# GRatTWCU/Social-STGCNN

Hardware: AMD Instinct MI355X
Metric: scene-windows/sec fwd+bwd (obs=8,pred=12) (higher is better)
Workload: dtype f32; 1 GPU; synthetic V=32 scene-windows, obs 8 / pred 12, batch 2048 per GPU, f32 (BASELINE north-star: V<=32, batch=2048; SURVEY 8d generator); global_batch=2048, step=aggregation + forward + bivariate NLL + backward + SGD update, parallelism=dp1

## Files before the change

social_stgcnn_amd/csrc/common.hpp:

```cpp
#pragma once
#include <hip/hip_runtime.h>
#include <cstdarg>
#include <cstdio>
#include <cstdint>

#include "../../include/stgcnn_hip.h"

namespace stg {

char *last_error_buf();
int fail(int code, const char *fmt, ...);
int hip_fail(hipError_t e, const char *what);

#define STG_REQUIRE(cond, code, ...)            \
    do {                                        \
        if (!(cond)) return stg::fail((code), __VA_ARGS__); \
    } while (0)

#define STG_LAUNCH_CHECK(what)                           \
    do {                                                 \
        hipError_t e_ = hipGetLastError();               \
        if (e_ != hipSuccess) return stg::hip_fail(e_, what); \
    } while (0)

static inline hipStream_t as_stream(void *s) { return reinterpret_cast<hipStream_t>(s); }
static inline bool aligned(const void *p, uintptr_t bytes) { return ((uintptr_t)p & (bytes - 1)) == 0; }

struct Launch {
    const char *what;
    dim3 grid, block;
    size_t lds;
    hipStream_t st;
    size_t raise_above = 0;
};
int raise_lds_limit(const void *kernel, size_t lds, const char *what);
template <typename... Params, typename... Args>
inline int launch(const Launch &l, void (*kernel)(Params...), const Args &...args) {
    if (l.lds > l.raise_above) {
        const int rc = raise_lds_limit(reinterpret_cast<const void *>(kernel), l.lds, l.what);
        if (rc != STG_OK) return rc;
    }
    hipLaunchKernelGGL(kernel, l.grid, l.block, l.lds, l.st, args...);
    STG_LAUNCH_CHECK(l.what);
    return STG_OK;
}

#ifdef STG_DIAG
int diag_env(const char *name, int dflt);
#define STG_SKIP(args, bit) (((args).debug_skip & (bit)) != 0)
#else
static inline int diag_env(const char *, int dflt) { return dflt; }
#define STG_SKIP(args, bit) false
#endif

__device__ __forceinline__ void stagger_start(int wave, int waves, int units) {
    if (waves >= 2 && wave >= waves / 2) {
        if (units == -1) __builtin_amdgcn_s_setprio(1);
        else if (units == -2) __builtin_amdgcn_s_setprio(2);
        else if (units <= -3) __builtin_amdgcn_s_setprio(3);
        for (int i = 0; i < units; ++i) __builtin_amdgcn_s_sleep(127);
    }
}

struct EventList {
    void **ev;
    int n, next;
    hipStream_t st;
    void mark() {
        if (ev && next < n) (void)hipEventRecord(reinterpret_cast<hipEvent_t>(ev[next]), st);
        ++next;
    }
    void finish() {
        while (ev && next < n) mark();
    }
};

constexpr int kWave = 64;
constexpr int kLdsBytes = 160 * 1024;
constexpr int kNumCU = 256;

template <int CTRL, int ROW_MASK = 0xf>
__device__ __forceinline__ void dpp_add(float &v) {
    v += __int_as_float(__builtin_amdgcn_update_dpp(0, __float_as_int(v), CTRL, ROW_MASK, 0xf, false));
}
__device__ __forceinline__ float wave_sum(float v) {
    dpp_add<0xB1>(v);
    dpp_add<0x4E>(v);
    dpp_add<0x141>(v);
    dpp_add<0x140>(v);
    dpp_add<0x142, 0xa>(v);
    dpp_add<0x143, 0xc>(v);
    return __int_as_float(__builtin_amdgcn_readlane(__float_as_int(v), 63));
}
template <int CTRL, int ROW_MASK = 0xf, int K>
__device__ __forceinline__ void dpp_stage(float (&v)[K]) {
#pragma unroll
    for (int k = 0; k < K; ++k) dpp_add<CTRL, ROW_MASK>(v[k]);
}
template <int K>
__device__ __forceinline__ void wave_sum_to_last(float (&v)[K]) {
    dpp_stage<0xB1>(v);
    dpp_stage<0x4E>(v);
    dpp_stage<0x141>(v);
    dpp_stage<0x140>(v);
    dpp_stage<0x142, 0xa>(v);
    dpp_stage<0x143, 0xc>(v);
}
template <int K>
__device__ __forceinline__ void wave_sum_n(float (&v)[K]) {
    wave_sum_to_last<K>(v);
#pragma unroll
    for (int k = 0; k < K; ++k) v[k] = __int_as_float(__builtin_amdgcn_readlane(__float_as_int(v[k]), 63));
}
__device__ __forceinline__ double wave_sum(double v) {
#pragma unroll
    for (int o = 32; o > 0; o >>= 1) v += __shfl_xor(v, o, 64);
    return v;
}

}
```

social_stgcnn_amd/csrc/scene_team.hpp:

```cpp
#pragma once
#include "common.hpp"

namespace stg {

__device__ __forceinline__ void team_barrier() { asm volatile("s_waitcnt lgkmcnt(0)\n\ts_barrier" ::: "memory"); }

struct SoloScene {
    static constexpr bool kTeam = false;
    int vi;
    __device__ __forceinline__ int w0() const { return 0; }
    __device__ __forceinline__ int wc() const { return vi; }
    __device__ __forceinline__ int nch() const { return 1; }
    __device__ __forceinline__ int ci() const { return 0; }
    __device__ __forceinline__ bool lead() const { return true; }
    __device__ __forceinline__ void sync() const { __builtin_amdgcn_wave_barrier(); }
    template <int K>
    __device__ __forceinline__ void sum(float (&v)[K], int) const { wave_sum_n<K>(v); }
    template <int K>
    __device__ __forceinline__ void reduce(float (&v)[K]) const { wave_sum_to_last<K>(v); }
    __device__ __forceinline__ bool writer() const { return (threadIdx.x & 63) == 63; }
    __device__ __forceinline__ float *row(float *scene_row) const { return scene_row; }
};

constexpr int kXrF_s1 = 0, kXrF_s2 = 20, kXrF_sm2 = 40, kXrF_sv2 = 80, kXrFwd = 120;
constexpr int kXrB_s1 = 0, kXrB_s3 = 64, kXrRows = 128;
constexpr int kTeamRow = 160;
constexpr int kTeamRowLoss = kTeamRow - 1;

struct TeamScene {
    static constexpr bool kTeam = true;
    int vi;
    int w0_, wc_;
    int nch_, ci_;
    float *xr;
    float *rows;
    bool bar;
    __device__ __forceinline__ int w0() const { return w0_; }
    __device__ __forceinline__ int wc() const { return wc_; }
    __device__ __forceinline__ int nch() const { return nch_; }
    __device__ __forceinline__ int ci() const { return ci_; }
    __device__ __forceinline__ bool lead() const { return ci_ == 0; }
    __device__ __forceinline__ void sync() const {
        if (bar) team_barrier();
        else __builtin_amdgcn_wave_barrier();
    }
    template <int K>
    __device__ __forceinline__ void sum(float (&v)[K], int slot) const {
        if (nch_ == 1) {
            wave_sum_n<K>(v);
            return;
        }
        wave_sum_to_last<K>(v);
        float *x = xr + slot;
        if ((threadIdx.x & 63) == 63) {
#pragma unroll
            for (int k = 0; k < K; ++k) x[ci_ * K + k] = v[k];
            if (nch_ == 2) {
#pragma unroll
                for (int k = 0; k < K; ++k) x[(ci_ + 2) * K + k] = 0.f;
            }
        }
        if (bar) team_barrier();
        float p[4][K];
#pragma unroll
        for (int c = 0; c < 4; ++c)
#pragma unroll
            for (int k = 0; k < K; ++k) p[c][k] = x[c * K + k];
#pragma unroll
        for (int k = 0; k < K; ++k) v[k] = (p[0][k] + p[1][k]) + (p[2][k] + p[3][k]);
    }
    template <int K>
    __device__ __forceinline__ void reduce(float (&v)[K]) const { wave_sum_to_last<K>(v); }
    __device__ __forceinline__ bool writer() const { return (threadIdx.x & 63) == 63; }
    __device__ __forceinline__ float *row(float *) const { return rows + ci_ * kTeamRow; }
    __device__ __forceinline__ const float *row_of(int c) const { return rows + c * kTeamRow; }
};

constexpr int kXrBwdWg = 2 * kXrRows + 4 * kTeamRow;

}
```

social_stgcnn_amd/csrc/txp_x6.hip:

```cpp
#include "txp_scene_common.hpp"
#include "nll_elem.hpp"
#include "txp_conv_bf16.hpp"

namespace stg {

namespace {

constexpr int C = Cfg::C, P = Cfg::P, T = Cfg::T;

constexpr int64_t kCanonAggStride32[2] = {(int64_t)(Cfg::CIN0 + 1) * Cfg::T * kCanonV, kCanonWs32};
constexpr int64_t kCanonAggAx32[2] = {0, kCanonLayout.ws_hdr_floats + (int64_t)kCanonLayout.blk[0].ws_ax * kCanonV};
constexpr int64_t kCanonAggCs32[2] = {(int64_t)Cfg::CIN0 * Cfg::T * kCanonV,
                                      kCanonLayout.ws_hdr_floats + (int64_t)kCanonLayout.blk[0].ws_cs * kCanonV};

template <Shape S, typename Args>
__device__ __forceinline__ void fold_shape(Args &a) {
    if constexpr (S != Shape::Generic) {
        ModelLayout k = kCanonLayout;
        k.eps = a.lay.eps;
        k.momentum = a.lay.momentum;
        k.bn_mode = a.lay.bn_mode;
        k.flags = a.lay.flags;
        k.wg_waves = a.lay.wg_waves;
        a.lay = k;
    }
    if constexpr (S == Shape::Canon32) {
        a.V = a.Vl = kCanonV;
        a.num_peds = nullptr;
        a.tier.order = nullptr;
        a.tier.key_start = nullptr;
        a.ws_stride = kCanonWs32;
    }
}
__device__ __forceinline__ unsigned canon32_code(int t, int nq) {
    return (unsigned)(cv::tile_row(kCanonV, t) << 8 | (cv::tile_col0(kCanonV, t) + nq));
}
template <Shape S>
__device__ __forceinline__ int lay_txp_b(const ModelLayout &L, int l) {
    if constexpr (S == Shape::Generic) return L.txp_b[l];
    else return kCanonLayout.txp_b[l];
}
template <Shape S>
__device__ __forceinline__ int lay_ws_z(const ModelLayout &L, int l) {
    if constexpr (S == Shape::Generic) return L.ws_z[l];
    else return kCanonLayout.ws_z[l];
}

#ifdef STG_DIAG
#define STG_X6_STAMP(a, n, k)                                                                                          \
    do {                                                                                                              \
        if ((a).stamps && (threadIdx.x & 63) == 0) (a).stamps[(int64_t)(n) * 16 + (k)] = __builtin_amdgcn_s_memrealtime(); \
    } while (0)
#else
#define STG_X6_STAMP(a, n, k) do { } while (0)
#endif

constexpr int kF6Tiles = 10, kF6Slots = 7;

__host__ __device__ inline int fwd6_region_floats(int v) { return (cv::image_bytes(v, kF6Slots) / 4 + 3) & ~3; }

template <bool BF, typename CK, Shape SH = Shape::Generic>
__device__ __forceinline__ void txp_fwd_scene_x6(const TxpFwdArgs &a, const float *__restrict__ params,
                                                 const float *blk_params, const float *blk_buffers, int n, int vi,
                                                 float *region, ptab_t *ptab, const CK &ck) {
    const ModelLayout &L = a.lay;
    const int V = a.V, lane = threadIdx.x & 63, nq = lane & 15, kq = lane >> 4;
    float *yn = a.y + (int64_t)n * (C * P) * V;
    if (vi < V)
        for (int e = lane + 64 * ck.ci(); e < C * P * (V - vi); e += 64 * ck.nch()) {
            const int r = e / (V - vi), w = vi + (e - r * (V - vi));
            yn[(int64_t)r * V + w] = 0.f;
        }
    if (vi == 0) return;
    const int npos = C * ck.wc(), ntiles = (npos + 15) >> 4;
    const float *Pm = params;
    float *wsn = a.ws ? a.ws + n * a.ws_stride : nullptr;
    float *statn = a.stats ? a.stats + (int64_t)n * L.stat_floats : nullptr;
    unsigned char *img = reinterpret_cast<unsigned char *>(region);
    const cv::LaneGeom lg = cv::lane_geom(vi, kF6Slots);
    constexpr bool bf16 = BF;
    const int SWs = save_sw(vi, bf16), VWs = save_vw(vi, bf16);

    {
        float sv[C * T / 2];
        const float *agn = a.agg + n * a.agg_stride;
        stgcn_block_fwd_cols<true, SH != Shape::Canon32>(a, blk_params, blk_buffers, L.blk[0], n, vi, wsn, statn,
                                                         agn + a.agg_ax, agn + a.agg_cs, nullptr, 0, region,
                                                         cv::image_bytes(vi, kF6Slots) >> 4, ptab, sv, ck);
        float *d2 = wsn ? wsn + ws_plane_off(L, V, 0) : nullptr;
        const int pl = lane & 31, pw = ck.w0() + pl, q = lane >> 5;
        if (pl < ck.wc()) {
#pragma unroll
            for (int row = 0; row < C; ++row) {
                const f32x4 v4 = {sv[row], sv[C + row], sv[2 * C + row], sv[3 * C + row]};
                cv::put4(img, (unsigned)(cv::pos_off(vi, 1 + row, pw) + 8 * q), lg.PL, v4);
                if (d2) {
                    store_vec4(d2, (row * SWs + pw + 1) * 3 + q, v4, bf16);
                    if (q == 0) store_vec4(d2, (row * SWs + pw + 1) * 3 + 2, f32x4{0.f, 0.f, 0.f, 0.f}, bf16);
                }
            }
        }
        if (wsn && lane < 2 * C * 3 && ck.lead()) {
            const int b = lane / 3, q = lane - b * 3, pos = (b >> 1) * SWs + ((b & 1) ? vi + 1 : 0);
            for (int l = 0; l <= L.L; ++l)
                store_vec4(wsn + ws_plane_off(L, V, l), pos * 3 + q, f32x4{0.f, 0.f, 0.f, 0.f}, bf16);
        }
    }
    ck.sync();

    if (STG_SKIP(a, 16)) return;
    const unsigned lds_base = (unsigned)(uintptr_t)img;
    [[maybe_unused]] cv::LaneBases lb;
    if constexpr (SH == Shape::Canon32) {
        static_assert(!CK::kTeam && 16 * kF6Tiles == C * kCanonV, "Canon32: one wave, ten full tiles");
        lb = cv::lane_bases(lds_base, lg, vi);
    }
    f32x4 av[kF6Tiles];
#pragma unroll
    for (int t = 0; t < kF6Tiles; ++t) av[t] = f32x4{0.f, 0.f, 0.f, 0.f};
    for (int l = 0; l <= L.L; ++l) {
        const bool is_out = l == L.L;
        cv::u32x4 w[cv::kWpVecs];
        cv::load_wp(a.wpf + (int64_t)l * cv::kWpDwords, w);
        const float *bias = Pm + (is_out ? L.out_b : lay_txp_b<SH>(L, l));
        f32x4 binit;
#pragma unroll
        for (int r = 0; r < 4; ++r) binit[r] = kq < 3 ? bias[4 * kq + r] : 0.f;
        const float alpha = is_out ? 0.f : Pm[L.prelus + l];
        float *zs = (wsn && !is_out) ? wsn + L.ws_hdr_floats + (int64_t)lay_ws_z<SH>(L, l) * V : nullptr;
        float *ps = (wsn && !is_out) ? wsn + ws_plane_off(L, V, l + 1) : nullptr;
        asm volatile("" ::"v"(w[0]), "v"(w[cv::kWpVecs - 1]), "v"(binit), "v"(alpha) : "memory");
        vm_drain();
        __builtin_amdgcn_s_setprio(1);
        auto finish = [&](int t, int h, int wc, bool ok, const f32x4 &z) __attribute__((always_inline)) {
            if (ok && kq < 3) {
                if (is_out) {
#pragma unroll
                    for (int r = 0; r < 4; ++r) yn[(int64_t)((4 * kq + r) * C + h) * V + wc] = z[r];
                } else {
                    f32x4 v4;
#pragma unroll
                    for (int r = 0; r < 4; ++r) v4[r] = (z[r] > 0.f ? z[r] : alpha * z[r]) + av[t][r];
                    av[t] = v4;
                    if (zs) {
                        store_vec4(zs, (h * VWs + wc) * 3 + kq, z, bf16);
                        store_vec4(ps, (h * SWs + wc + 1) * 3 + kq, v4, bf16);
                    }
                }
            }
        };
        if constexpr (SH == Shape::Canon32) {
            cv::for_tiles<kF6Tiles>([&](auto tc) __attribute__((always_inline)) {
                constexpr int t = decltype(tc)::value;
                cv::BHalf b;
                f32x4 z = binit;
                cv::load_b_half_imm<0, kCanonV, t>(lb, b);
                cv::mma_half<0>(w, b, z);
                cv::load_b_half_imm<1, kCanonV, t>(lb, b);
                cv::mma_half<1>(w, b, z);
                finish(t, cv::tile_row(kCanonV, t), cv::tile_col0(kCanonV, t) + nq, true, z);
            });
        } else {
            unsigned code = cv::tile_code(0, ptab, npos);
#pragma unroll
            for (int t = 0; t < kF6Tiles; ++t) {
                if (t < ntiles) {
                    const cv::Tile tl = cv::tile_from<1>(t, code, npos, lg, vi);
                    if (t + 1 < kF6Tiles) code = cv::tile_code(t + 1, ptab, npos);
                    cv::BHalf b;
                    f32x4 z = binit;
                    cv::load_b_half<0>(lds_base, tl, b);
                    cv::mma_half<0>(w, b, z);
                    cv::load_b_half<1>(lds_base, tl, b);
                    cv::mma_half<1>(w, b, z);
                    finish(t, tl.h, tl.w, tl.ok, z);
                }
            }
        }
        __builtin_amdgcn_s_setprio(0);
        if (is_out) break;
        ck.sync();
        unsigned codes[kF6Tiles];
#pragma unroll
        for (int t = 0; t < kF6Tiles; ++t) codes[t] = SH == Shape::Canon32 ? canon32_code(t, nq) : cv::tile_code(t, ptab, npos);
#pragma unroll
        for (int t = 0; t < kF6Tiles; ++t) {
            const int p = 16 * t + nq;
            if (p < npos && kq < 3) {
                const unsigned hw = codes[t];
                cv::put4(img, (unsigned)(cv::pos_off(vi, 1 + (int)(hw >> 8), (int)(hw & 0xffu)) + 8 * kq), lg.PL, av[t]);
            }
        }
        ck.sync();
    }
}

template <int WPB, bool BF, Shape S>
__global__ __launch_bounds__(WPB * 64, WPB == 8 ? 1 : 2) __attribute__((amdgpu_waves_per_eu(2, 2))) void txp_fwd_x6_kernel(
    const TxpFwdArgs a0, const float *__restrict__ params, const float *__restrict__ buffers) {
    extern __shared__ __attribute__((aligned(16))) float sm[];
    TxpFwdArgs a = a0;
    fold_shape<S>(a);
    if constexpr (S == Shape::Canon32) {
        const int w = a.ws != nullptr;
        a.agg_stride = kCanonAggStride32[w];
        a.agg_ax = kCanonAggAx32[w];
        a.agg_cs = kCanonAggCs32[w];
    }
    const int Vl = a.Vl, wave = threadIdx.x >> 6;
    const int per_wave = fwd6_region_floats(Vl) + ptab_floats(Vl);
    float *region = sm + wave * per_wave;
    ptab_t *ptab = reinterpret_cast<ptab_t *>(region + fwd6_region_floats(Vl));
    float *blk_p = sm + WPB * per_wave, *blk_b = blk_p + ((a.lay.n_blk_params + 3) & ~3);
    stage_block_params(a.lay, params, buffers, blk_p, blk_b, WPB * 64);
    const int gw = __builtin_amdgcn_readfirstlane(blockIdx.x * WPB + wave), nw = gridDim.x * WPB;
    int begin, end;
    tier_range(a.tier, a.N, a.V, begin, end);
    const int M = end - begin;
    for (int r = 0; r * nw < M; ++r) {
        const int it = walk_item(r, gw, nw, M, a.tier.order != nullptr && a.tier.serpentine);
        if (it < 0) continue;
        const int n = __builtin_amdgcn_readfirstlane(a.tier.order ? scene_index(a.tier.order[begin + it], a.N) : it);
        int vi = a.num_peds ? a.num_peds[n] : a.V;
        vi = __builtin_amdgcn_readfirstlane(vi < 0 ? 0 : (vi > a.V ? a.V : vi));
        STG_X6_STAMP(a, n, 0);
        txp_fwd_scene_x6<BF, SoloScene, S>(a, params, blk_p, blk_b, n, vi, region, ptab, SoloScene{vi});
        __builtin_amdgcn_wave_barrier();
        STG_X6_STAMP(a, n, 8);
    }
}

constexpr int kX6Tiles = 10;
constexpr int kX6Slots = 7;
__host__ __device__ inline int bwd6_region_floats(int v) {
    const int img = cv::image_bytes(v, kX6Slots) / 4, tail = (2 * C * (T + 2) + C * T) * v;
    return ((img > tail ? img : tail) + 3) & ~3;
}

template <bool BF, typename CK, Shape SH = Shape::Generic>
__device__ __forceinline__ void txp_bwd_scene_x6(const TxpBwdArgs &a, const float *blk_params, int n, int vi, float *region,
                                                 ptab_t *ptab, const CK &ck) {
    const ModelLayout &L = a.lay;
    const int V = a.V, lane = threadIdx.x & 63, nq = lane & 15, kq = lane >> 4;
    float *slope_row = a.rows + (int64_t)n * (L.n_blk_params + L.n_txp) + L.n_blk_params;
    if (vi == 0) {
        for (int e = lane; e < L.n_blk_params + L.n_txp; e += 64) slope_row[e - L.n_blk_params] = 0.f;
        if (a.nll_target && lane == 0) a.nll_losses[n] = 0.f;
        return;
    }
    const int npos = C * ck.wc(), ntiles = (npos + 15) >> 4;
    const float *Pm = a.params;
    const float *wsn = a.ws + n * a.ws_stride;
    const float *dyn = a.dy + (int64_t)n * (C * P) * V;
    float *prow = ck.row(slope_row - L.n_blk_params);
    if constexpr (CK::kTeam) {
        for (int e = lane; e < kTeamRow; e += 64) prow[e] = 0.f;
    }
    unsigned char *img = reinterpret_cast<unsigned char *>(region);
    const cv::LaneGeom lg = cv::lane_geom(vi, kX6Slots);
    constexpr bool bf16 = BF;
    const int VWs = save_vw(vi, bf16);
    auto tile_slots = [&](int t, int &rec, int &quad) {
        if constexpr (SH == Shape::Canon32) {
            const int h = cv::tile_row(kCanonV, t), w = cv::tile_col0(kCanonV, t) + nq;
            quad = (h * VWs + w) * 3 + kq;
            rec = cv::pos_off(vi, 1 + h, w) + 8 * kq;
        } else {
            const int p = 16 * t + nq;
            const unsigned hw = ptab[p < npos ? p : 0];
            const int h = (int)(hw >> 8), w = (int)(hw & 0xffu);
            quad = (h * VWs + w) * 3 + kq;
            rec = (p < npos && kq < 3) ? cv::pos_off(vi, 1 + h, w) + 8 * kq : -1;
        }
    };
    auto has_quad = [&](int rec) { return SH == Shape::Canon32 ? kq < 3 : rec >= 0; };
    {
        uint4 *z4 = reinterpret_cast<uint4 *>(img);
        for (int e = lane + 64 * ck.ci(); e < cv::image_bytes(vi, kX6Slots) >> 4; e += 64 * ck.nch()) z4[e] = make_uint4(0u, 0u, 0u, 0u);
    }
    [[maybe_unused]] cv::LaneBases lb;
    if constexpr (SH == Shape::Canon32) {
        static_assert(!CK::kTeam && 16 * kX6Tiles == C * kCanonV, "Canon32: one wave, ten full tiles");
        lb = cv::lane_bases((unsigned)(uintptr_t)img, lg, vi);
    } else {
        build_ptab(ptab, ck.w0(), ck.wc());
    }
    ck.sync();
    f32x4 dcur[kX6Tiles];
#pragma unroll
    for (int t = 0; t < kX6Tiles; ++t) dcur[t] = f32x4{0.f, 0.f, 0.f, 0.f};

    for (int l = L.L; l >= 0; --l) {
        float *dzo = a.dzg + ((int64_t)n * (L.L + 1) + l) * dz_slot(V);
        if (STG_SKIP(a, 512) || (l == L.L && STG_SKIP(a, 2048)) || (l != L.L && STG_SKIP(a, 4096))) {
        } else if (l == L.L) {
            const int wcw = ck.wc();
            const int vp = wcw <= 1 ? 1 : (wcw <= 2 ? 2 : (wcw <= 4 ? 4 : (wcw <= 8 ? 8 : (wcw <= 16 ? 16 : 32))));
            const int sh = __builtin_ctz(vp), rpi = 64 >> sh;
            const int sub = lane >> sh, wl = lane & (vp - 1), w = ck.w0() + wl;
            const bool okw = wl < wcw;
            float *S = reinterpret_cast<float *>(img + lg.PL);
            auto put1 = [&](int rc, float g) { S[rc * vi + w] = g; };
            if (a.nll_target) {
                const float *tn = a.nll_target + (int64_t)n * P * V * 2;
                const float inv_cnt = 1.0f / (float)(P * vi);
                const float gs = inv_cnt * (a.nll_weights ? a.nll_weights[n] : 1.f);
                float lacc = 0.f;
#pragma unroll 1
                for (int p0 = 0; p0 < P; p0 += rpi) {
                    const int p = p0 + sub;
                    if (okw && p < P) {
                        const float *q = dyn + (int64_t)p * V + w;
                        const float2 tg = *reinterpret_cast<const float2 *>(tn + ((int64_t)p * V + w) * 2);
                        float g[5];
#ifdef STG_DIAG
                        if (STG_SKIP(a, 1 << 21))
                            lacc += nll_elem_t<true>(q[0], q[(int64_t)P * V], q[(int64_t)2 * P * V], q[(int64_t)3 * P * V],
                                                     q[(int64_t)4 * P * V], tg.x, tg.y, true, g);
                        else
#endif
                        lacc += nll_elem(q[0], q[(int64_t)P * V], q[(int64_t)2 * P * V], q[(int64_t)3 * P * V],
                                         q[(int64_t)4 * P * V], tg.x, tg.y, true, g);
#pragma unroll
                        for (int f = 0; f < C; ++f) put1(f * P + p, g[f] * gs);
                    }
                }
                float ls[1] = {lacc};
                ck.template reduce<1>(ls);
                if (ck.writer()) {
                    if constexpr (CK::kTeam) prow[kTeamRowLoss] = ls[0];
                    else a.nll_losses[n] = ls[0] * inv_cnt;
                }
            } else {
                constexpr int U = 4;
#pragma unroll 1
                for (int r0 = 0; r0 < C * P; r0 += rpi * U) {
                    float dv[U];
#pragma unroll
                    for (int u = 0; u < U; ++u) {
                        const int row = r0 + u * rpi + sub;
                        dv[u] = (okw && row < C * P) ? dyn[(int64_t)row * V + w] : 0.f;
                    }
#pragma unroll
                    for (int u = 0; u < U; ++u) {
                        const int row = r0 + u * rpi + sub;
                        if (okw && row < C * P) put1(row, dv[u]);
                    }
                }
            }
            __builtin_amdgcn_wave_barrier();
            vm_drain();
            f32x4 (&qd)[kX6Tiles] = dcur;
#pragma unroll
            for (int t = 0; t < kX6Tiles; ++t) {
                const int p = 16 * t + nq;
                const unsigned hw = SH == Shape::Canon32 ? canon32_code(t, nq) : ptab[p < npos ? p : 0];
                const float *sq = S + ((4 * (kq < 3 ? kq : 0)) * C + (int)(hw >> 8)) * vi + (int)(hw & 0xffu);
                qd[t] = f32x4{sq[0], sq[C * vi], sq[2 * C * vi], sq[3 * C * vi]};
            }
            ck.sync();
            {
                uint4 *z4 = reinterpret_cast<uint4 *>(img + lg.PL);
                for (int e = lane + 64 * ck.ci(); e < (2 * lg.PL + 128) >> 4; e += 64 * ck.nch()) z4[e] = make_uint4(0u, 0u, 0u, 0u);
            }
            ck.sync();
            int rec[kX6Tiles], qv[kX6Tiles];
#pragma unroll
            for (int t = 0; t < kX6Tiles; ++t) tile_slots(t, rec[t], qv[t]);
#pragma unroll
            for (int t = 0; t < kX6Tiles; ++t) {
                if (has_quad(rec[t])) {
                    cv::put4(img, (unsigned)rec[t], lg.PL, qd[t]);
                    store_vec4(dzo, qv[t], qd[t], bf16);
                }
            }
        } else {
            const float *zl = wsn + L.ws_hdr_floats + (int64_t)lay_ws_z<SH>(L, l) * V;
            const float alpha = Pm[L.prelus + l];
            float slope_acc = 0.f;
            f32x4 zv[kX6Tiles];
            int rec[kX6Tiles], qv[kX6Tiles];
#pragma unroll
            for (int t = 0; t < kX6Tiles; ++t) tile_slots(t, rec[t], qv[t]);
#pragma unroll
            for (int t = 0; t < kX6Tiles; ++t)
                zv[t] = has_quad(rec[t]) ? load_vec4_raw(zl, qv[t], bf16) : f32x4{1.f, 1.f, 1.f, 1.f};
            asm volatile("" ::"v"(zv[0]), "v"(zv[1]), "v"(zv[2]), "v"(zv[3]), "v"(zv[4]), "v"(zv[5]), "v"(zv[6]), "v"(zv[7]),
                         "v"(zv[8]), "v"(zv[9]), "v"(alpha)
                         : "memory");
            vm_drain();
#pragma unroll
            for (int t = 0; t < kX6Tiles; ++t) {
                if (has_quad(rec[t])) {
                    f32x4 dzv;
                    const f32x4 zq = finish_vec4(zv[t], bf16);
#pragma unroll
                    for (int r = 0; r < 4; ++r) {
                        const float z = zq[r], d = dcur[t][r];
                        float dz = d;
                        if (!(z > 0.f)) {
                            dz = alpha * d;
                            slope_acc = fmaf(d, z, slope_acc);
                        }
                        dzv[r] = dz;
                    }
                    cv::put4(img, (unsigned)rec[t], lg.PL, dzv);
                    store_vec4(dzo, qv[t], dzv, bf16);
                }
            }
            float ss[1] = {slope_acc};
            ck.template reduce<1>(ss);
            if (ck.writer()) prow[L.n_blk_params + l] = ss[0];
        }
        ck.sync();
        if (!STG_SKIP(a, 1024)) {
            cv::u32x4 w[cv::kWpVecs];
            cv::load_wp(a.wp + (int64_t)l * cv::kWpDwords, w);
            asm volatile("" ::"v"(w[0]), "v"(w[cv::kWpVecs - 1]) : "memory");
            vm_drain();
            const unsigned lds_base = (unsigned)(uintptr_t)img;
            const bool keep = l != L.L && l != 0;
            const f32x4 zero = {0.f, 0.f, 0.f, 0.f};
            if constexpr (SH == Shape::Canon32) {
                cv::for_tiles<kX6Tiles>([&](auto tc) __attribute__((always_inline)) {
                    constexpr int t = decltype(tc)::value;
                    cv::BHalf b;
                    f32x4 acc = keep ? dcur[t] : zero;
                    cv::load_b_half_imm<0, kCanonV, t>(lb, b);
                    cv::mma_half<0>(w, b, acc);
                    cv::load_b_half_imm<1, kCanonV, t>(lb, b);
                    cv::mma_half<1>(w, b, acc);
                    dcur[t] = acc;
                });
            } else {
                unsigned code = cv::tile_code(0, ptab, npos);
#pragma unroll
                for (int t = 0; t < kX6Tiles; ++t) {
                    if (t < ntiles) {
                        const cv::Tile tl = cv::tile_from<1>(t, code, npos, lg, vi);
                        if (t + 1 < kX6Tiles) code = cv::tile_code(t + 1, ptab, npos);
                        cv::BHalf b;
                        f32x4 acc = keep ? dcur[t] : zero;
                        cv::load_b_half<0>(lds_base, tl, b);
                        cv::mma_half<0>(w, b, acc);
                        cv::load_b_half<1>(lds_base, tl, b);
                        cv::mma_half<1>(w, b, acc);
                        dcur[t] = acc;
                    }
                }
            }
        }
        ck.sync();
    }
    float *D = region;
#pragma unroll
    for (int t = 0; t < kX6Tiles; ++t) {
        const int p = 16 * t + nq;
        if (p < npos && kq < T / 4) {
            const unsigned hw = SH == Shape::Canon32 ? canon32_code(t, nq) : ptab[p];
            const int h = (int)(hw >> 8), ww = (int)(hw & 0xffu);
#pragma unroll
            for (int r = 0; r < 4; ++r) D[((4 * kq + r) * C + h) * vi + ww] = dcur[t][r];
        }
    }
    __builtin_amdgcn_wave_barrier();
    if constexpr (!CK::kTeam) {
        for (int e = L.L + lane; e < L.n_txp; e += 64) slope_row[e] = 0.f;
    }
    if (!STG_SKIP(a, 4))
        stgcn_block_bwd_cols<true>(a, blk_params, L.blk[0], n, vi, D, slope_row - L.n_blk_params, a.ws + n * a.ws_stride, ck);
    if constexpr (CK::kTeam) {
        ck.sync();
        if (ck.lead()) {
            float *row = slope_row - L.n_blk_params;
            const int nrow = L.n_blk_params + L.n_txp;
            for (int e0 = 0; e0 < kTeamRow; e0 += 64) {
                const int e = e0 + lane < kTeamRow ? e0 + lane : kTeamRow - 2;
                float t = ck.row_of(0)[e];
                for (int c = 1; c < ck.nch(); ++c) t += ck.row_of(c)[e];
                if (e < nrow) row[e] = t;
                if (e == kTeamRowLoss && a.nll_target) a.nll_losses[n] = t * (1.0f / (float)(P * vi));
            }
        }
    }
}

template <int WPB, bool BF, Shape S>
__global__ __launch_bounds__(WPB * 64, WPB == 8 ? 1 : 2) __attribute__((amdgpu_waves_per_eu(2, 2))) void txp_bwd_x6_kernel(
    const TxpBwdArgs a0) {
    extern __shared__ __attribute__((aligned(16))) float sm[];
    TxpBwdArgs a = a0;
    fold_shape<S>(a);
    const int Vl = a.Vl, wave = threadIdx.x >> 6;
    const int per_wave = bwd6_region_floats(Vl) + bwd_ptab_floats(Vl);
    float *region = sm + wave * per_wave;
    ptab_t *ptab = reinterpret_cast<ptab_t *>(region + bwd6_region_floats(Vl));
    float *blk_p = sm + WPB * per_wave;
    stage_block_params(a.lay, a.params, nullptr, blk_p, nullptr, WPB * 64);
    const int gw = __builtin_amdgcn_readfirstlane(blockIdx.x * WPB + wave), nw = gridDim.x * WPB;
    int begin, end;
    tier_range(a.tier, a.N, a.V, begin, end);
    const int M = end - begin;
    for (int r = 0; r * nw < M; ++r) {
        const int it = walk_item(r, gw, nw, M, a.tier.order != nullptr && a.tier.serpentine);
        if (it < 0) continue;
        const int n = __builtin_amdgcn_readfirstlane(a.tier.order ? scene_index(a.tier.order[begin + it], a.N) : it);
        int vi = a.num_peds ? a.num_peds[n] : a.V;
        vi = __builtin_amdgcn_readfirstlane(vi < 0 ? 0 : (vi > a.V ? a.V : vi));
        STG_X6_STAMP(a, n, 0);
        txp_bwd_scene_x6<BF, SoloScene, S>(a, blk_p, n, vi, region, ptab, SoloScene{vi});
        __builtin_amdgcn_wave_barrier();
        STG_X6_STAMP(a, n, 8);
    }
}

__host__ __device__ inline int step6_per_wave_floats(int v) {
    const int f = fwd6_region_floats(v) + ptab_floats(v), b = bwd6_region_floats(v) + bwd_ptab_floats(v);
    return f > b ? f : b;
}

template <int WPB, bool BF>
__global__ __launch_bounds__(WPB * 64, 2) __attribute__((amdgpu_waves_per_eu(2, 2))) void txp_step_x6_kernel(
    const TxpFwdArgs f0, const TxpBwdArgs b0) {
    constexpr Shape S = Shape::Canon32;
    extern __shared__ __attribute__((aligned(16))) float sm[];
    TxpFwdArgs f = f0;
    fold_shape<S>(f);
    f.agg_stride = kCanonAggStride32[1];
    f.agg_ax = kCanonAggAx32[1];
    f.agg_cs = kCanonAggCs32[1];
    TxpBwdArgs b = b0;
    fold_shape<S>(b);
    const int wave = threadIdx.x >> 6;
    const int per_wave = step6_per_wave_floats(kCanonV);
    float *region = sm + wave * per_wave;
    ptab_t *ptab = reinterpret_cast<ptab_t *>(region + bwd6_region_floats(kCanonV));
    float *blk_p = sm + WPB * per_wave, *blk_b = blk_p + ((kCanonLayout.n_blk_params + 3) & ~3);
    stage_block_params(f.lay, f.params, f.buffers, blk_p, blk_b, WPB * 64);
    const int n = __builtin_amdgcn_readfirstlane(blockIdx.x * WPB + wave);
    if (n >= f.N) return;
    STG_X6_STAMP(f, n, 0);
    txp_fwd_scene_x6<BF, SoloScene, S>(f, f.params, blk_p, blk_b, n, kCanonV, region, ptab, SoloScene{kCanonV});
    __builtin_amdgcn_fence(__ATOMIC_RELEASE, "wavefront");
    __builtin_amdgcn_wave_barrier();
    __builtin_amdgcn_fence(__ATOMIC_ACQUIRE, "wavefront");
    STG_X6_STAMP(f, n, 8);
    STG_X6_STAMP(b, n, 0);
    txp_bwd_scene_x6<BF, SoloScene, S>(b, blk_p, n, kCanonV, region, ptab, SoloScene{kCanonV});
    __builtin_amdgcn_wave_barrier();
    STG_X6_STAMP(b, n, 8);
}

struct TeamCount {
    int n4, n2, n1;
    int u4, u2, units;
    bool sorted;
};
__device__ __forceinline__ TeamCount team_count(const SceneTier &t, const TeamGeom &g, const int32_t *num_peds, int N, int V) {
    TeamCount c;
    c.sorted = t.order && t.key_start;
    if (c.sorted) {
        const int a4 = g.v2 < V ? t.key_start[V - g.v2] : 0, a2 = g.v1 < V ? t.key_start[V - g.v1] : 0;
        c.n4 = a4;
        c.n2 = a2 - a4;
        c.u2 = (c.n2 + 1) >> 1;
    } else {
        const bool pairs = !num_peds && V > g.v1 && V <= g.v2;
        c.n4 = (V > g.v1 && !pairs) ? N : 0;
        c.n2 = pairs ? N : 0;
        c.u2 = (c.n2 + 1) >> 1;
    }
    c.n1 = N - c.n4 - c.n2;
    c.u4 = c.n4;
    c.units = c.u4 + c.u2 + ((c.n1 + 3) >> 2);
    return c;
}
struct TeamUnit {
    int n, vi;
    int nch, ci, slot;
    int w0, wc;
};
__device__ __forceinline__ TeamUnit team_unit(const SceneTier &t, const TeamCount &c, const int32_t *__restrict__ num_peds,
                                              int N, int V, int u) {
    const int wave = __builtin_amdgcn_readfirstlane(threadIdx.x >> 6);
    TeamUnit q;
    int idx;
    if (u < c.u4) {
        q.nch = 4; q.slot = 0; q.ci = wave; idx = u;
    } else if (u < c.u4 + c.u2) {
        const int i0 = c.n4 + 2 * (u - c.u4);
        if (i0 + 1 < c.n4 + c.n2) { q.nch = 2; q.slot = wave >> 1; q.ci = wave & 1; idx = i0 + q.slot; }
        else { q.nch = 4; q.slot = 0; q.ci = wave; idx = i0; }
    } else {
        q.nch = 1; q.slot = wave; q.ci = 0; idx = c.n4 + c.n2 + 4 * (u - c.u4 - c.u2) + wave;
    }
    q.n = idx < N ? (c.sorted ? scene_index(t.order[idx], N) : idx) : -1;
    q.n = __builtin_amdgcn_readfirstlane(q.n);
    int vi = q.n >= 0 ? (num_peds ? num_peds[q.n] : V) : 0;
    vi = __builtin_amdgcn_readfirstlane(vi < 0 ? 0 : (vi > V ? V : vi));
    q.vi = vi;
    const int wc = (vi + q.nch - 1) / q.nch;
    q.w0 = q.ci * wc;
    q.wc = vi - q.w0 < wc ? (vi - q.w0 > 0 ? vi - q.w0 : 0) : wc;
    return q;
}
__device__ __forceinline__ int team_workers(int units, int grid) {
    const int rounds = (units + grid - 1) / grid;
    return rounds > 0 ? (units + rounds - 1) / rounds : 1;
}
__host__ __device__ inline int team_ptab_floats() { return ptab_floats(32); }

template <bool BF>
__global__ __launch_bounds__(256, 2) __attribute__((amdgpu_waves_per_eu(2, 2))) void txp_fwd_team_kernel(
    const TxpFwdArgs a, const float *__restrict__ params, const float *__restrict__ buffers) {
    extern __shared__ __attribute__((aligned(16))) float sm[];
    const int wave = __builtin_amdgcn_readfirstlane(threadIdx.x >> 6);
    const int R = a.team.region_floats;
    ptab_t *ptab = reinterpret_cast<ptab_t *>(sm + R + wave * team_ptab_floats());
    float *xr = sm + R + 4 * team_ptab_floats();
    float *blk_p = xr + 2 * kXrFwd, *blk_b = blk_p + ((a.lay.n_blk_params + 3) & ~3);
    stage_block_params(a.lay, params, buffers, blk_p, blk_b, 256);
    const TeamCount tc = team_count(a.tier, a.team, a.num_peds, a.N, a.V);
    const int G = team_workers(tc.units, gridDim.x);
    int prev = 1;
    for (int r = 0; r * G < tc.units; ++r) {
        const int u = walk_item(r, blockIdx.x, G, tc.units, a.tier.serpentine != 0);
        if (u < 0 || (int)blockIdx.x >= G) continue;
        const TeamUnit q = team_unit(a.tier, tc, a.num_peds, a.N, a.V, u);
        if (q.nch > 1 || prev > 1) team_barrier();
        prev = q.nch;
        if (q.n >= 0) {
            const TeamScene ck{q.vi, q.w0, q.wc, q.nch, q.ci, xr + (q.slot & 1) * kXrFwd, nullptr, q.nch > 1 && !STG_SKIP(a, 1 << 20)};
            float *region = sm + q.slot * ((R >> 2) * q.nch);
            txp_fwd_scene_x6<BF>(a, params, blk_p, blk_b, q.n, q.vi, region, ptab, ck);
        }
        __builtin_amdgcn_wave_barrier();
    }
}

template <bool BF>
__global__ __launch_bounds__(256, 2) __attribute__((amdgpu_waves_per_eu(2, 2))) void txp_bwd_team_kernel(const TxpBwdArgs a) {
    extern __shared__ __attribute__((aligned(16))) float sm[];
    const int wave = __builtin_amdgcn_readfirstlane(threadIdx.x >> 6);
    const int R = a.team.region_floats;
    ptab_t *ptab = reinterpret_cast<ptab_t *>(sm + R + wave * team_ptab_floats());
    float *xr = sm + R + 4 * team_ptab_floats();
    float *blk_p = xr + kXrBwdWg;
    stage_block_params(a.lay, a.params, nullptr, blk_p, nullptr, 256);
    const TeamCount tc = team_count(a.tier, a.team, a.num_peds, a.N, a.V);
    const int G = team_workers(tc.units, gridDim.x);
    int prev = 1;
    for (int r = 0; r * G < tc.units; ++r) {
        const int u = walk_item(r, blockIdx.x, G, tc.units, a.tier.serpentine != 0);
        if (u < 0 || (int)blockIdx.x >= G) continue;
        const TeamUnit q = team_unit(a.tier, tc, a.num_peds, a.N, a.V, u);
        if (q.nch > 1 || prev > 1) team_barrier();
        prev = q.nch;
        if (q.n >= 0) {
            const TeamScene ck{q.vi, q.w0, q.wc, q.nch, q.ci, xr + (q.slot & 1) * kXrRows,
                               xr + 2 * kXrRows + q.slot * q.nch * kTeamRow, q.nch > 1 && !STG_SKIP(a, 1 << 20)};
            float *region = sm + q.slot * ((R >> 2) * q.nch);
            txp_bwd_scene_x6<BF>(a, blk_p, q.n, q.vi, region, ptab, ck);
        }
        __builtin_amdgcn_wave_barrier();
    }
}

}

bool txp_fwd_x6_fits(const ModelLayout &L, int V) {
    return L.n_txp > 0 && V <= kTeamMaxV && !(L.flags & STG_OPT_F32_MFMA) && L.n_blocks == 1 &&
           L.blk[0].cin == Cfg::CIN0 && !diag_env("STG_FWD_F32", 0);
}

constexpr int kTeamFineBatch = 1536, kTeamFinestBatch = 384;
static int team_waves(int v, int v1, int v2) { return v <= v1 ? 1 : (v <= v2 ? 2 : 4); }
static bool team_geom(int N, int V, bool uniform, TeamGeom *g) {
    g->on = 0;
    if (V > kTeamMaxV) return false;
    int v1 = 32, v2 = 64;
    if (N < kTeamFinestBatch) { v1 = 8; v2 = 16; }
    else if (N < kTeamFineBatch) { v1 = 16; v2 = 32; }
    if (uniform)
        while (v1 < 32 && (int64_t)N * team_waves(V, v1, v2) > 2048) { v1 *= 2; v2 *= 2; }
    if (const int e = diag_env("STG_TEAM_V1", 0)) v1 = e;
    if (const int e = diag_env("STG_TEAM_V2", 0)) v2 = e;
    if (v1 > 32) v1 = 32;
    if (v2 > 64) v2 = 64;
    if (v2 < v1) v2 = v1;
    auto region = [&](int v) { return fwd6_region_floats(v); };
    int r = 4 * region(v1 < V ? v1 : V);
    if (2 * region(v2 < V ? v2 : V) > r) r = 2 * region(v2 < V ? v2 : V);
    if (region(V) > r) r = region(V);
    g->on = 1; g->v1 = v1; g->v2 = v2; g->region_floats = (r + 15) & ~15;
    return true;
}
static bool team_wanted(int N, int V, bool uniform, TeamGeom *g) {
    if (!team_geom(N, V, uniform, g)) return false;
    return V > 16 * kF6Tiles / C || g->v1 < V || diag_env("STG_TEAM", 0) != 0;
}
static int team_grid(size_t lds_bytes, int N) {
    int per_cu = (int)(kLdsBytes / lds_bytes);
    if (per_cu > 2) per_cu = 2;
    if (per_cu < 1) per_cu = 1;
    const int g = kNumCU * per_cu;
    return g < N ? g : N;
}

template <typename Args>
static Shape canon_shape(const Args &a, bool *ok) {
    *ok = true;
    if (!is_canonical(a.lay)) return Shape::Generic;
    if (a.num_peds || a.V != kCanonV) return Shape::Canon;
    *ok = a.Vl == kCanonV && !a.tier.order && !a.tier.key_start && a.ws_stride == kCanonWs32;
    return Shape::Canon32;
}
static bool canon32_agg_matches(const TxpFwdArgs &a) {
    const int w = a.ws != nullptr;
    return a.agg_stride == kCanonAggStride32[w] && a.agg_ax == kCanonAggAx32[w] && a.agg_cs == kCanonAggCs32[w];
}

template <int W>
static auto fwd_x6_kernel(bool bf, Shape sh) {
    if (bf) return sh == Shape::Canon32 ? txp_fwd_x6_kernel<W, true, Shape::Canon32> : txp_fwd_x6_kernel<W, true, Shape::Generic>;
    if (sh == Shape::Canon32) return txp_fwd_x6_kernel<W, false, Shape::Canon32>;
    return sh == Shape::Canon ? txp_fwd_x6_kernel<W, false, Shape::Canon> : txp_fwd_x6_kernel<W, false, Shape::Generic>;
}
template <int W>
static auto bwd_x6_kernel(bool bf, Shape sh) {
    if (bf) {
        if (sh == Shape::Canon32) return txp_bwd_x6_kernel<W, true, Shape::Canon32>;
        return sh == Shape::Canon ? txp_bwd_x6_kernel<W, true, Shape::Canon> : txp_bwd_x6_kernel<W, true, Shape::Generic>;
    }
    if (sh == Shape::Canon32) return txp_bwd_x6_kernel<W, false, Shape::Canon32>;
    return sh == Shape::Canon ? txp_bwd_x6_kernel<W, false, Shape::Canon> : txp_bwd_x6_kernel<W, false, Shape::Generic>;
}

int launch_txp_fwd_x6(const TxpFwdArgs &a0, hipStream_t st) {
    TxpFwdArgs a = a0;
    STG_REQUIRE(a.wpf, STG_EINVAL, "txp_fwd_x6: the prepared operands are missing");
    const bool bf = (a.lay.flags & STG_OPT_BF16_STORE) != 0;
    if (team_wanted(a.N, a.V, a.num_peds == nullptr, &a.team)) {
        const size_t lds = ((size_t)a.team.region_floats + 4 * team_ptab_floats() + 2 * kXrFwd + wave_param_floats(a.lay)) * sizeof(float);
        STG_REQUIRE(lds <= (size_t)kLdsBytes, STG_ELDS, "txp_fwd_team: V=%d needs %zu bytes of LDS", a.V, lds);
        return launch(Launch{"txp_fwd_team", dim3(team_grid(lds, a.N)), dim3(256), lds, st},
                      bf ? txp_fwd_team_kernel<true> : txp_fwd_team_kernel<false>, a, a.params, a.buffers);
    }
    STG_REQUIRE(a.V <= 16 * kF6Tiles / C, STG_EUNSUPPORTED, "txp_fwd_x6: V=%d outside the exact-bf16 kernels", a.V);
    const size_t per_wave = (size_t)(fwd6_region_floats(a.Vl) + ptab_floats(a.Vl)) * sizeof(float);
    const int wpb = wave_wpb(per_wave) == 8 ? 8 : 4;
    const size_t lds = per_wave * wpb + wave_param_floats(a.lay) * sizeof(float);
    bool ok;
    const Shape sh = canon_shape(a, &ok);
    STG_REQUIRE(ok && (sh != Shape::Canon32 || canon32_agg_matches(a)), STG_EINVAL,
                "txp_fwd_x6: the canonical V=%d batch does not match its compiled layout", a.V);
    return launch(Launch{"txp_fwd_x6", dim3(wave_grid(lds, wpb, a.N)), dim3(wpb * 64), lds, st},
                  wpb == 8 ? fwd_x6_kernel<8>(bf, sh) : fwd_x6_kernel<4>(bf, sh), a, a.params, a.buffers);
}

bool txp_bwd_x6_fits(const ModelLayout &L, int V) {
    return L.n_txp > 0 && V <= kTeamMaxV && L.n_blocks == 1 && L.blk[0].cin == Cfg::CIN0 &&
           !(L.flags & (STG_OPT_SPLIT_BF16 | STG_OPT_F32_MFMA)) && !diag_env("STG_BWD_F32", 0);
}
int64_t txp_bwd_x6_wp_floats(const ModelLayout &L) { return (int64_t)(L.L + 1) * cv::kWpDwords; }
int launch_txp_bwd_x6(const TxpBwdArgs &a0, hipStream_t st) {
    TxpBwdArgs a = a0;
    STG_REQUIRE(a.wp, STG_EINVAL, "txp_bwd_x6: the prepared operands are missing");
    const bool bf = (a.lay.flags & STG_OPT_BF16_STORE) != 0;
    if (team_wanted(a.N, a.V, a.num_peds == nullptr, &a.team)) {
        const size_t lds = ((size_t)a.team.region_floats + 4 * team_ptab_floats() + kXrBwdWg + wave_param_floats(a.lay)) * sizeof(float);
        STG_REQUIRE(lds <= (size_t)kLdsBytes, STG_ELDS, "txp_bwd_team: V=%d needs %zu bytes of LDS", a.V, lds);
        return launch(Launch{"txp_bwd_team", dim3(team_grid(lds, a.N)), dim3(256), lds, st},
                      bf ? txp_bwd_team_kernel<true> : txp_bwd_team_kernel<false>, a);
    }
    STG_REQUIRE(a.V <= 16 * kX6Tiles / C, STG_EUNSUPPORTED, "txp_bwd_x6: V=%d outside the exact-bf16 kernels", a.V);
    const size_t per_wave = (size_t)(bwd6_region_floats(a.Vl) + bwd_ptab_floats(a.Vl)) * sizeof(float);
    const int wpb = wave_wpb(per_wave) == 8 ? 8 : 4;
    const size_t lds = per_wave * wpb + wave_param_floats(a.lay) * sizeof(float);
    bool ok;
    const Shape sh = canon_shape(a, &ok);
    STG_REQUIRE(ok, STG_EINVAL, "txp_bwd_x6: the canonical V=%d batch does not match its compiled layout", a.V);
    return launch(Launch{"txp_bwd_x6", dim3(wave_grid(lds, wpb, a.N)), dim3(wpb * 64), lds, st},
                  wpb == 8 ? bwd_x6_kernel<8>(bf, sh) : bwd_x6_kernel<4>(bf, sh), a);
}

static bool step_x6_plain(int debug_skip_f, int debug_skip_b, int stagger_f, int stagger_b) {
    const size_t pf = (size_t)(fwd6_region_floats(kCanonV) + ptab_floats(kCanonV)) * sizeof(float);
    const size_t pb = (size_t)(bwd6_region_floats(kCanonV) + bwd_ptab_floats(kCanonV)) * sizeof(float);
    return !debug_skip_f && !debug_skip_b && !stagger_f && !stagger_b && wave_wpb(pf) != 8 && wave_wpb(pb) != 8;
}
bool txp_step_x6_fits(const ModelLayout &L, const int32_t *num_peds, int N, int V) {
    TeamGeom g;
    const int skip = diag_env("STG_DEBUG_SKIP", 0);
    return is_canonical(L) && V == kCanonV && !num_peds && txp_fwd_x6_fits(L, V) && txp_bwd_x6_fits(L, V) &&
           !team_wanted(N, V, true, &g) &&
           step_x6_plain(skip, skip, diag_env("STG_STAGGER_F", 0), diag_env("STG_STAGGER_B", 0));
}
static bool txp_step_x6_applies(const TxpFwdArgs &f, const TxpBwdArgs &b) {
    if (!f.wpf || !b.wp || !f.ws || f.ws != b.ws || f.N != b.N || f.V != b.V || f.params != b.params) return false;
    if (f.lay.flags != b.lay.flags || !step_x6_plain(f.debug_skip, b.debug_skip, f.stagger, b.stagger)) return false;
    TeamGeom g;
    if (team_wanted(f.N, f.V, f.num_peds == nullptr, &g) || team_wanted(b.N, b.V, b.num_peds == nullptr, &g)) return false;
    bool okf, okb;
    if (canon_shape(f, &okf) != Shape::Canon32 || canon_shape(b, &okb) != Shape::Canon32) return false;
    return okf && okb && canon32_agg_matches(f);
}
int launch_txp_step_x6(const TxpFwdArgs &f, const TxpBwdArgs &b, hipStream_t st) {
    STG_REQUIRE(txp_step_x6_applies(f, b), STG_EINVAL, "txp_step_x6: the batch is outside the one-launch scene kernel");
    constexpr int wpb = 4;
    const size_t lds = ((size_t)step6_per_wave_floats(kCanonV) * wpb + wave_param_floats(f.lay)) * sizeof(float);
    const bool bf = (f.lay.flags & STG_OPT_BF16_STORE) != 0;
    STG_REQUIRE(2 * lds <= (size_t)kLdsBytes, STG_ELDS, "txp_step_x6: %zu bytes of LDS do not fit two workgroups per CU", lds);
    return launch(Launch{"txp_step_x6", dim3((f.N + wpb - 1) / wpb), dim3(wpb * 64), lds, st},
                  bf ? txp_step_x6_kernel<wpb, true> : txp_step_x6_kernel<wpb, false>, f, b);
}

}
```

Baseline: 10.86 million scene-windows/s.

## Hand off forward outputs through LDS in fused step kernel; inline-asm DPP wave sums

In the one-launch Canon32 step kernel, the forward pass now also writes its output tile into the LDS scratch image. The backward pass reads predictions from there for the NLL gradient instead of re-reading them from global memory, and only zeroes the part of the image it still needs. Separately, wave reductions for Canon32 solo scenes use hand-written batched v_add_f32_dpp inline assembly with a single s_nop per stage rather than per-value builtins. The assembly path relies on correct hazard padding, and the hand-off assumes P is even and that LDS regions do not overlap.

```diff
diff --git a/social_stgcnn_amd/csrc/common.hpp b/social_stgcnn_amd/csrc/common.hpp
--- a/social_stgcnn_amd/csrc/common.hpp
+++ b/social_stgcnn_amd/csrc/common.hpp
@@ -97,18 +97,83 @@
 #pragma unroll
     for (int k = 0; k < K; ++k) dpp_add<CTRL, ROW_MASK>(v[k]);
 }
-template <int K>
+#define STG_DPP_I(i, c) "v_add_f32_dpp %" #i ", %" #i ", %" #i " " c "\n\t"
+#define STG_DPP_I1(c) STG_DPP_I(0, c)
+#define STG_DPP_I5(c) STG_DPP_I1(c) STG_DPP_I(1, c) STG_DPP_I(2, c) STG_DPP_I(3, c) STG_DPP_I(4, c)
+#define STG_DPP_I10(c) STG_DPP_I5(c) STG_DPP_I(5, c) STG_DPP_I(6, c) STG_DPP_I(7, c) STG_DPP_I(8, c) STG_DPP_I(9, c)
+#define STG_DPP_I15(c) STG_DPP_I10(c) STG_DPP_I(10, c) STG_DPP_I(11, c) STG_DPP_I(12, c) STG_DPP_I(13, c) STG_DPP_I(14, c)
+#define STG_DPP_I16(c) STG_DPP_I15(c) STG_DPP_I(15, c)
+#define STG_DPP_I25(c)                                                                                               \
+    STG_DPP_I16(c) STG_DPP_I(16, c) STG_DPP_I(17, c) STG_DPP_I(18, c) STG_DPP_I(19, c) STG_DPP_I(20, c) STG_DPP_I(21, c) \
+        STG_DPP_I(22, c) STG_DPP_I(23, c) STG_DPP_I(24, c)
+#define STG_DPP_V(v, i) "+v"((v)[O + (i)])
+#define STG_DPP_V1(v) STG_DPP_V(v, 0)
+#define STG_DPP_V5(v) STG_DPP_V1(v), STG_DPP_V(v, 1), STG_DPP_V(v, 2), STG_DPP_V(v, 3), STG_DPP_V(v, 4)
+#define STG_DPP_V10(v) STG_DPP_V5(v), STG_DPP_V(v, 5), STG_DPP_V(v, 6), STG_DPP_V(v, 7), STG_DPP_V(v, 8), STG_DPP_V(v, 9)
+#define STG_DPP_V15(v) STG_DPP_V10(v), STG_DPP_V(v, 10), STG_DPP_V(v, 11), STG_DPP_V(v, 12), STG_DPP_V(v, 13), STG_DPP_V(v, 14)
+#define STG_DPP_V16(v) STG_DPP_V15(v), STG_DPP_V(v, 15)
+#define STG_DPP_V25(v)                                                                                               \
+    STG_DPP_V16(v), STG_DPP_V(v, 16), STG_DPP_V(v, 17), STG_DPP_V(v, 18), STG_DPP_V(v, 19), STG_DPP_V(v, 20), STG_DPP_V(v, 21), \
+        STG_DPP_V(v, 22), STG_DPP_V(v, 23), STG_DPP_V(v, 24)
+#define STG_DPP_STMT(v, c)                                                       \
+    do {                                                                         \
+        if constexpr (N == 25) asm("s_nop 1\n\t" STG_DPP_I25(c) : STG_DPP_V25(v)); \
+        else if constexpr (N == 16) asm("s_nop 1\n\t" STG_DPP_I16(c) : STG_DPP_V16(v)); \
+        else if constexpr (N == 15) asm("s_nop 1\n\t" STG_DPP_I15(c) : STG_DPP_V15(v)); \
+        else if constexpr (N == 10) asm("s_nop 1\n\t" STG_DPP_I10(c) : STG_DPP_V10(v)); \
+        else if constexpr (N == 5) asm("s_nop 1\n\t" STG_DPP_I5(c) : STG_DPP_V5(v)); \
+        else asm("s_nop 1\n\t" STG_DPP_I1(c) : STG_DPP_V1(v));                   \
+    } while (0)
+template <int S, int O = 0, int K>
+__device__ __forceinline__ void wave_sum_stage(float (&v)[K]) {
+    constexpr int R = K - O;
+    constexpr int N = R >= 25 ? 25 : (R >= 16 ? 16 : (R >= 15 ? 15 : (R >= 10 ? 10 : (R >= 5 ? 5 : 1))));
+    static_assert(S >= 0 && S < 6 && R >= 1, "six stages, at least one value");
+    if constexpr (S == 0) STG_DPP_STMT(v, "quad_perm:[1,0,3,2] row_mask:0xf bank_mask:0xf");
+    else if constexpr (S == 1) STG_DPP_STMT(v, "quad_perm:[2,3,0,1] row_mask:0xf bank_mask:0xf");
+    else if constexpr (S == 2) STG_DPP_STMT(v, "row_half_mirror row_mask:0xf bank_mask:0xf");
+    else if constexpr (S == 3) STG_DPP_STMT(v, "row_mirror row_mask:0xf bank_mask:0xf");
+    else if constexpr (S == 4) STG_DPP_STMT(v, "row_bcast:15 row_mask:0xa bank_mask:0xf");
+    else STG_DPP_STMT(v, "row_bcast:31 row_mask:0xc bank_mask:0xf");
+    if constexpr (R > N) wave_sum_stage<S, O + N>(v);
+}
+#undef STG_DPP_STMT
+#undef STG_DPP_V25
+#undef STG_DPP_V16
+#undef STG_DPP_V15
+#undef STG_DPP_V10
+#undef STG_DPP_V5
+#undef STG_DPP_V1
+#undef STG_DPP_V
+#undef STG_DPP_I25
+#undef STG_DPP_I16
+#undef STG_DPP_I15
+#undef STG_DPP_I10
+#undef STG_DPP_I5
+#undef STG_DPP_I1
+#undef STG_DPP_I
+
+template <int K, bool ASM = false>
 __device__ __forceinline__ void wave_sum_to_last(float (&v)[K]) {
-    dpp_stage<0xB1>(v);
-    dpp_stage<0x4E>(v);
-    dpp_stage<0x141>(v);
-    dpp_stage<0x140>(v);
-    dpp_stage<0x142, 0xa>(v);
-    dpp_stage<0x143, 0xc>(v);
+    if constexpr (ASM) {
+        wave_sum_stage<0>(v);
+        wave_sum_stage<1>(v);
+        wave_sum_stage<2>(v);
+        wave_sum_stage<3>(v);
+        wave_sum_stage<4>(v);
+        wave_sum_stage<5>(v);
+    } else {
+        dpp_stage<0xB1>(v);
+        dpp_stage<0x4E>(v);
+        dpp_stage<0x141>(v);
+        dpp_stage<0x140>(v);
+        dpp_stage<0x142, 0xa>(v);
+        dpp_stage<0x143, 0xc>(v);
+    }
 }
-template <int K>
+template <int K, bool ASM = false>
 __device__ __forceinline__ void wave_sum_n(float (&v)[K]) {
-    wave_sum_to_last<K>(v);
+    wave_sum_to_last<K, ASM>(v);
 #pragma unroll
     for (int k = 0; k < K; ++k) v[k] = __int_as_float(__builtin_amdgcn_readlane(__float_as_int(v[k]), 63));
 }
diff --git a/social_stgcnn_amd/csrc/scene_team.hpp b/social_stgcnn_amd/csrc/scene_team.hpp
--- a/social_stgcnn_amd/csrc/scene_team.hpp
+++ b/social_stgcnn_amd/csrc/scene_team.hpp
@@ -5,7 +5,8 @@
 
 __device__ __forceinline__ void team_barrier() { asm volatile("s_waitcnt lgkmcnt(0)\n\ts_barrier" ::: "memory"); }
 
-struct SoloScene {
+template <bool DPP_ASM>
+struct SoloSceneT {
     static constexpr bool kTeam = false;
     int vi;
     __device__ __forceinline__ int w0() const { return 0; }
@@ -15,12 +16,13 @@
     __device__ __forceinline__ bool lead() const { return true; }
     __device__ __forceinline__ void sync() const { __builtin_amdgcn_wave_barrier(); }
     template <int K>
-    __device__ __forceinline__ void sum(float (&v)[K], int) const { wave_sum_n<K>(v); }
+    __device__ __forceinline__ void sum(float (&v)[K], int) const { wave_sum_n<K, DPP_ASM>(v); }
     template <int K>
-    __device__ __forceinline__ void reduce(float (&v)[K]) const { wave_sum_to_last<K>(v); }
+    __device__ __forceinline__ void reduce(float (&v)[K]) const { wave_sum_to_last<K, DPP_ASM>(v); }
     __device__ __forceinline__ bool writer() const { return (threadIdx.x & 63) == 63; }
     __device__ __forceinline__ float *row(float *scene_row) const { return scene_row; }
 };
+using SoloScene = SoloSceneT<false>;
 
 constexpr int kXrF_s1 = 0, kXrF_s2 = 20, kXrF_sm2 = 40, kXrF_sv2 = 80, kXrFwd = 120;
 constexpr int kXrB_s1 = 0, kXrB_s3 = 64, kXrRows = 128;
diff --git a/social_stgcnn_amd/csrc/txp_x6.hip b/social_stgcnn_amd/csrc/txp_x6.hip
--- a/social_stgcnn_amd/csrc/txp_x6.hip
+++ b/social_stgcnn_amd/csrc/txp_x6.hip
@@ -32,6 +32,13 @@
         a.ws_stride = kCanonWs32;
     }
 }
+#ifdef STG_WAVE_SUM_BUILTIN
+constexpr bool kWaveSumAsm = false;
+#else
+constexpr bool kWaveSumAsm = true;
+#endif
+template <Shape S>
+using SoloOf = SoloSceneT<S == Shape::Canon32 && kWaveSumAsm>;
 __device__ __forceinline__ unsigned canon32_code(int t, int nq) {
     return (unsigned)(cv::tile_row(kCanonV, t) << 8 | (cv::tile_col0(kCanonV, t) + nq));
 }
@@ -59,7 +66,7 @@
 
 __host__ __device__ inline int fwd6_region_floats(int v) { return (cv::image_bytes(v, kF6Slots) / 4 + 3) & ~3; }
 
-template <bool BF, typename CK, Shape SH = Shape::Generic>
+template <bool BF, typename CK, Shape SH = Shape::Generic, bool HO = false>
 __device__ __forceinline__ void txp_fwd_scene_x6(const TxpFwdArgs &a, const float *__restrict__ params,
                                                  const float *blk_params, const float *blk_buffers, int n, int vi,
                                                  float *region, ptab_t *ptab, const CK &ck) {
@@ -137,6 +144,7 @@
                 if (is_out) {
 #pragma unroll
                     for (int r = 0; r < 4; ++r) yn[(int64_t)((4 * kq + r) * C + h) * V + wc] = z[r];
+                    if constexpr (HO) av[t] = z;
                 } else {
                     f32x4 v4;
 #pragma unroll
@@ -178,6 +186,17 @@
             }
         }
         __builtin_amdgcn_s_setprio(0);
+        if constexpr (HO) {
+            static_assert(!HO || SH == Shape::Canon32, "the hand-off is the one-launch Canon32 kernel's");
+            if (is_out && kq < 3) {
+                float *S = reinterpret_cast<float *>(img + lg.PL);
+#pragma unroll
+                for (int t = 0; t < kF6Tiles; ++t)
+#pragma unroll
+                    for (int r = 0; r < 4; ++r)
+                        S[((4 * kq + r) * C + cv::tile_row(kCanonV, t)) * kCanonV + cv::tile_col0(kCanonV, t) + nq] = av[t][r];
+            }
+        }
         if (is_out) break;
         ck.sync();
         unsigned codes[kF6Tiles];
@@ -224,7 +243,7 @@
         int vi = a.num_peds ? a.num_peds[n] : a.V;
         vi = __builtin_amdgcn_readfirstlane(vi < 0 ? 0 : (vi > a.V ? a.V : vi));
         STG_X6_STAMP(a, n, 0);
-        txp_fwd_scene_x6<BF, SoloScene, S>(a, params, blk_p, blk_b, n, vi, region, ptab, SoloScene{vi});
+        txp_fwd_scene_x6<BF, SoloOf<S>, S>(a, params, blk_p, blk_b, n, vi, region, ptab, SoloOf<S>{vi});
         __builtin_amdgcn_wave_barrier();
         STG_X6_STAMP(a, n, 8);
     }
@@ -237,7 +256,7 @@
     return ((img > tail ? img : tail) + 3) & ~3;
 }
 
-template <bool BF, typename CK, Shape SH = Shape::Generic>
+template <bool BF, typename CK, Shape SH = Shape::Generic, bool HO = false>
 __device__ __forceinline__ void txp_bwd_scene_x6(const TxpBwdArgs &a, const float *blk_params, int n, int vi, float *region,
                                                  ptab_t *ptab, const CK &ck) {
     const ModelLayout &L = a.lay;
@@ -275,8 +294,10 @@
     };
     auto has_quad = [&](int rec) { return SH == Shape::Canon32 ? kq < 3 : rec >= 0; };
     {
+        static_assert(!HO || SH == Shape::Canon32, "the hand-off is the one-launch Canon32 kernel's");
         uint4 *z4 = reinterpret_cast<uint4 *>(img);
-        for (int e = lane + 64 * ck.ci(); e < cv::image_bytes(vi, kX6Slots) >> 4; e += 64 * ck.nch()) z4[e] = make_uint4(0u, 0u, 0u, 0u);
+        const int zero_bytes = HO ? lg.PL : cv::image_bytes(vi, kX6Slots);
+        for (int e = lane + 64 * ck.ci(); e < zero_bytes >> 4; e += 64 * ck.nch()) z4[e] = make_uint4(0u, 0u, 0u, 0u);
     }
     [[maybe_unused]] cv::LaneBases lb;
     if constexpr (SH == Shape::Canon32) {
@@ -306,8 +327,23 @@
                 const float inv_cnt = 1.0f / (float)(P * vi);
                 const float gs = inv_cnt * (a.nll_weights ? a.nll_weights[n] : 1.f);
                 float lacc = 0.f;
+                if constexpr (HO) {
+                    static_assert(!HO || P % 2 == 0, "two prediction steps per round");
+                    const float2 *tq = reinterpret_cast<const float2 *>(tn) + sub * V + w;
+                    float2 tg = tq[0];
 #pragma unroll 1
-                for (int p0 = 0; p0 < P; p0 += rpi) {
+                    for (int i = 0; i < P / 2; ++i) {
+                        const float2 tg_next = tq[(i + 1 < P / 2 ? i + 1 : i) * 2 * V];
+                        float *q = S + (2 * i + sub) * vi + w;
+                        float g[5];
+                        lacc += nll_elem(q[0], q[P * vi], q[2 * P * vi], q[3 * P * vi], q[4 * P * vi], tg.x, tg.y, true, g);
+#pragma unroll
+                        for (int f = 0; f < C; ++f) q[f * P * vi] = g[f] * gs;
+                        tg = tg_next;
+                    }
+                }
+#pragma unroll 1
+                for (int p0 = 0; p0 < (HO ? 0 : P); p0 += rpi) {
                     const int p = p0 + sub;
                     if (okw && p < P) {
                         const float *q = dyn + (int64_t)p * V + w;
@@ -508,7 +544,7 @@
         int vi = a.num_peds ? a.num_peds[n] : a.V;
         vi = __builtin_amdgcn_readfirstlane(vi < 0 ? 0 : (vi > a.V ? a.V : vi));
         STG_X6_STAMP(a, n, 0);
-        txp_bwd_scene_x6<BF, SoloScene, S>(a, blk_p, n, vi, region, ptab, SoloScene{vi});
+        txp_bwd_scene_x6<BF, SoloOf<S>, S>(a, blk_p, n, vi, region, ptab, SoloOf<S>{vi});
         __builtin_amdgcn_wave_barrier();
         STG_X6_STAMP(a, n, 8);
     }
@@ -519,6 +555,11 @@
     return f > b ? f : b;
 }
 
+#ifdef STG_NO_STEP_HANDOFF
+constexpr bool kStepHandoff = false;
+#else
+constexpr bool kStepHandoff = true;
+#endif
 template <int WPB, bool BF>
 __global__ __launch_bounds__(WPB * 64, 2) __attribute__((amdgpu_waves_per_eu(2, 2))) void txp_step_x6_kernel(
     const TxpFwdArgs f0, const TxpBwdArgs b0) {
@@ -540,13 +581,13 @@
     const int n = __builtin_amdgcn_readfirstlane(blockIdx.x * WPB + wave);
     if (n >= f.N) return;
     STG_X6_STAMP(f, n, 0);
-    txp_fwd_scene_x6<BF, SoloScene, S>(f, f.params, blk_p, blk_b, n, kCanonV, region, ptab, SoloScene{kCanonV});
+    txp_fwd_scene_x6<BF, SoloOf<S>, S, kStepHandoff>(f, f.params, blk_p, blk_b, n, kCanonV, region, ptab, SoloOf<S>{kCanonV});
     __builtin_amdgcn_fence(__ATOMIC_RELEASE, "wavefront");
     __builtin_amdgcn_wave_barrier();
     __builtin_amdgcn_fence(__ATOMIC_ACQUIRE, "wavefront");
     STG_X6_STAMP(f, n, 8);
     STG_X6_STAMP(b, n, 0);
-    txp_bwd_scene_x6<BF, SoloScene, S>(b, blk_p, n, kCanonV, region, ptab, SoloScene{kCanonV});
+    txp_bwd_scene_x6<BF, SoloOf<S>, S, kStepHandoff>(b, blk_p, n, kCanonV, region, ptab, SoloOf<S>{kCanonV});
     __builtin_amdgcn_wave_barrier();
     STG_X6_STAMP(b, n, 8);
 }
```

Result: no change. 10.94 million scene-windows/s, median of 6 (+0.8%).
